# HeyWeCome/WhisprRec

Measured on AMD Instinct MI355X. Metric: BPR training triplets/sec, higher is better.
Workload: dtype f32; 1 GPU; BPRMF emb_size=64, synthetic 1000000 users x 1000000 items (uniform ids), batch 65536, SGD l2=0, plan build in timed region; batch=65536, emb_size=64, optimizer=SGD, plan_chunk_batches=64, tables=single GPU, step_stream=whisprrec_amd.hip_ops.PipelinedSgd, plan=group plan (no per-batch sort: flags + lists of the shared rows, wr_group.hip), chained_step_launch=True, plan_build=on a side stream, beside the steps of the chunk before

## Files before the change

whisprrec_amd/csrc/wr_group.hip:

```cpp
#include "wr_common.h"
#include <hip/hip_ext.h>

#include <algorithm>

namespace wr {

constexpr int kGpThreads = 1024;
constexpr unsigned kGpRangeBits = 18;
constexpr int kGpWords = 1 << (kGpRangeBits - 5);
constexpr int kGpCap = 8192;
constexpr int kGpBins = 4096;
constexpr int kGpMaxBin = 256;
constexpr int kGpMaxRanges = 8;
constexpr int64_t kGpMaxBatch = 1 << 17;
constexpr int kGpLongRun = 64;
constexpr int kGpMetaWords = 16;
#ifndef WR_GP_DBG
#define WR_GP_DBG 0
#endif

struct GroupLayout {
    int64_t nb, B, fw;
    int R_u, R_i, cap_u, cap_i;
    unsigned mask_u, mask_i, hbits_u, hbits_i;
    int64_t flags, ucnt, icnt, ul_row, ul_src, il_row, il_src, total;
    int64_t zero_words;
};

static inline int ranges_for(int64_t n_rows, unsigned *mask, unsigned *hbits, int *cap) {
    unsigned bits = kGpRangeBits;
    while (bits < kGpRangeBits + 3 && (int64_t(1) << bits) < n_rows) ++bits;
    *mask = (1u << bits) - 1u;
    *hbits = bits;
    const int R = 1 << (bits - kGpRangeBits);
    *cap = kGpCap;
    return R;
}

static bool group_layout(int64_t n, int64_t B, int64_t n_users, int64_t n_items, GroupLayout &L) {
    if (n <= 0 || n >= (int64_t(1) << 31) || B <= 0 || B > kGpMaxBatch) return false;
    if (n_users <= 0 || n_users >= (int64_t(1) << 31) || n_items <= 0 || n_items >= (int64_t(1) << 31)) return false;
    L.nb = (n + B - 1) / B;
    L.B = B;
    L.fw = (B + 31) / 32;
    L.R_u = ranges_for(n_users, &L.mask_u, &L.hbits_u, &L.cap_u);
    L.R_i = ranges_for(n_items, &L.mask_i, &L.hbits_i, &L.cap_i);
    L.flags = kGpMetaWords;
    L.ucnt = L.flags + L.nb * L.fw * 4;
    L.icnt = L.ucnt + align_up(L.nb * L.R_u, 4);
    L.zero_words = L.icnt + align_up(L.nb * L.R_i, 4);
    L.ul_row = L.zero_words;
    L.ul_src = L.ul_row + L.nb * L.R_u * (int64_t)L.cap_u;
    L.il_row = L.ul_src + L.nb * L.R_u * (int64_t)L.cap_u;
    L.il_src = L.il_row + L.nb * L.R_i * (int64_t)L.cap_i;
    L.total = L.il_src + L.nb * L.R_i * (int64_t)L.cap_i;
    return true;
}

struct GpDev {
    int *meta;
    unsigned *flags;
    int *ucnt, *icnt;
    int *ul_row, *ul_src, *il_row, *il_src;
    int R_u, R_i, cap_u, cap_i;
    unsigned mask_u, mask_i, hbits_u, hbits_i;
    int fw;
};

static inline GpDev group_dev(int32_t *plan, const GroupLayout &L) {
    return GpDev{plan, reinterpret_cast<unsigned *>(plan + L.flags), plan + L.ucnt, plan + L.icnt, plan + L.ul_row,
                 plan + L.ul_src, plan + L.il_row, plan + L.il_src, L.R_u, L.R_i, L.cap_u, L.cap_i, L.mask_u, L.mask_i,
                 L.hbits_u, L.hbits_i, (int)L.fw};
}

template <typename F>
__device__ __forceinline__ void gp_scan(const int *__restrict__ a, int cnt, F f) {
    if ((reinterpret_cast<uintptr_t>(a) & 15u) == 0) {
        const int n4 = cnt >> 2;
        const int4 *a4 = reinterpret_cast<const int4 *>(a);
        int i = threadIdx.x;
        for (; i + 3 * kGpThreads < n4; i += 4 * kGpThreads) {
            int4 v[4];
#pragma unroll
            for (int q = 0; q < 4; ++q) v[q] = a4[i + q * kGpThreads];
#pragma unroll
            for (int q = 0; q < 4; ++q) {
                const int at = 4 * (i + q * kGpThreads);
                f(v[q].x, at);
                f(v[q].y, at + 1);
                f(v[q].z, at + 2);
                f(v[q].w, at + 3);
            }
        }
        for (; i < n4; i += kGpThreads) {
            const int4 v = a4[i];
            f(v.x, 4 * i);
            f(v.y, 4 * i + 1);
            f(v.z, 4 * i + 2);
            f(v.w, 4 * i + 3);
        }
        for (int j = (n4 << 2) + threadIdx.x; j < cnt; j += kGpThreads) f(a[j], j);
    } else {
        for (int j = threadIdx.x; j < cnt; j += kGpThreads) f(a[j], j);
    }
}

__global__ __launch_bounds__(kGpThreads) void group_plan_kernel(const int *__restrict__ u, const int *__restrict__ p,
                                                                 const int *__restrict__ n, int64_t n_total, int B, int nb,
                                                                 int n_users, int n_items, GpDev L) {
    extern __shared__ __attribute__((aligned(16))) unsigned gp_lds[];
    unsigned *seen = gp_lds;
    unsigned long long *keys = reinterpret_cast<unsigned long long *>(gp_lds);
    unsigned *multi = gp_lds + 2 * kGpCap;
    unsigned *f0 = multi + kGpWords, *f1 = f0 + L.fw, *f2 = f1 + L.fw;
    int &n_list = *reinterpret_cast<int *>(f2 + L.fw);
    const int per = L.R_u + L.R_i;
    const unsigned lb = xcd_contiguous_id(blockIdx.x, gridDim.x);
    const int b = (int)(lb / (unsigned)per), rr = (int)(lb % (unsigned)per);
    const bool item = rr >= L.R_u;
    const unsigned r = (unsigned)(item ? rr - L.R_u : rr);
    const int64_t base = (int64_t)b * B;
    const int Bb = (int)((base + B <= n_total) ? B : (n_total - base));
    const unsigned n_rows = (unsigned)(item ? n_items : n_users);
    const unsigned mask = item ? L.mask_i : L.mask_u;
    const unsigned rb = (item ? L.hbits_i : L.hbits_u) - kGpRangeBits, rsel = (1u << rb) - 1u;
    for (int i = threadIdx.x; i < kGpWords; i += kGpThreads) {
        seen[i] = 0u;
        multi[i] = 0u;
    }
    for (int i = threadIdx.x; i < 3 * L.fw; i += kGpThreads) f0[i] = 0u;
    if (threadIdx.x == 0) n_list = 0;
    __syncthreads();
    auto mark = [&](int row, int) {
        if ((unsigned)row >= n_rows) {
            L.meta[0] = 1;
            return;
        }
        const unsigned h = (unsigned)row & mask;
        if ((h & rsel) != r) return;
        const unsigned bit = h >> rb, m = 1u << (bit & 31u);
        const unsigned old = atomicOr(&seen[bit >> 5], m);
        if (old & m) atomicOr(&multi[bit >> 5], m);
    };
    if (!(WR_GP_DBG & 8)) {
        if (item) {
            gp_scan(p + base, Bb, mark);
            gp_scan(n + base, Bb, mark);
        } else {
            gp_scan(u + base, Bb, mark);
        }
    }
    __syncthreads();
    auto several = [&](int row) -> bool {
        const unsigned h = (unsigned)row & mask;
        if ((h & rsel) != r) return false;
        const unsigned bit = h >> rb;
        return (multi[bit >> 5] >> (bit & 31u)) & 1u;
    };
    auto append = [&](int row, unsigned src) {
        const int pos = atomicAdd(&n_list, 1);
        if (pos < kGpCap) keys[pos] = ((unsigned long long)(unsigned)row << 32) | src;
    };
    if (!(WR_GP_DBG & 2)) {
        const bool next = b + 1 < nb && !(WR_GP_DBG & 16);
        const int64_t nbase = base + B;
        const int Bn = next ? (int)((nbase + B <= n_total) ? B : (n_total - nbase)) : 0;
        auto defer = [&](int row, int t) {
            if (several(row)) atomicOr(&f2[t >> 5], 1u << (t & 31));
        };
        if (item) {
            gp_scan(p + base, Bb, [&](int row, int t) {
                if (several(row)) {
                    atomicOr(&f0[t >> 5], 1u << (t & 31));
                    append(row, (unsigned)t << 1);
                }
            });
            gp_scan(n + base, Bb, [&](int row, int t) {
                if (several(row)) {
                    atomicOr(&f1[t >> 5], 1u << (t & 31));
                    append(row, ((unsigned)t << 1) | 1u);
                }
            });
            gp_scan(p + nbase, Bn, defer);
            gp_scan(n + nbase, Bn, defer);
        } else {
            gp_scan(u + base, Bb, [&](int row, int t) {
                if (several(row)) {
                    atomicOr(&f0[t >> 5], 1u << (t & 31));
                    append(row, (unsigned)t << 1);
                }
            });
            gp_scan(u + nbase, Bn, defer);
        }
    }
    __syncthreads();
    if (!(WR_GP_DBG & 4)) {
        unsigned *fb = L.flags + (int64_t)b * L.fw * 4;
        for (int w = threadIdx.x; w < L.fw; w += kGpThreads) {
            if (f0[w]) __hip_atomic_fetch_or(fb + 4 * w + (item ? 1 : 0), f0[w], __ATOMIC_RELAXED, __HIP_MEMORY_SCOPE_AGENT);
            if (item && f1[w]) __hip_atomic_fetch_or(fb + 4 * w + 2, f1[w], __ATOMIC_RELAXED, __HIP_MEMORY_SCOPE_AGENT);
            if (f2[w])
                __hip_atomic_fetch_or(fb + 4 * (L.fw + w) + 3, f2[w], __ATOMIC_RELAXED, __HIP_MEMORY_SCOPE_AGENT);
        }
    }
    const int cap = item ? L.cap_i : L.cap_u, R = item ? L.R_i : L.R_u;
    int m = n_list;
    if (m > cap) {
        if (threadIdx.x == 0) L.meta[1] = 1;
        m = cap;
    }
    int *cnt = reinterpret_cast<int *>(multi);
    unsigned short *out16 = reinterpret_cast<unsigned short *>(multi + kGpBins);
    int *wave_tot = reinterpret_cast<int *>(f0);
    auto bin_of = [&](unsigned long long k) -> int { return (int)(((((unsigned)(k >> 32)) & mask) >> rb) & (kGpBins - 1)); };
    int *lrow = (item ? L.il_row : L.ul_row) + ((int64_t)b * R + r) * cap, *lsrc = (item ? L.il_src : L.ul_src) + ((int64_t)b * R + r) * cap;
    __syncthreads();
    for (int i = threadIdx.x; i < kGpBins; i += kGpThreads) cnt[i] = 0;
    __syncthreads();
    if (!(WR_GP_DBG & 1)) {
        for (int j = threadIdx.x; j < m; j += kGpThreads) atomicAdd(&cnt[bin_of(keys[j])], 1);
        __syncthreads();
        constexpr int kOwn = kGpBins / kGpThreads;
        const int c0 = (int)threadIdx.x * kOwn;
        int local = 0;
#pragma unroll
        for (int j = 0; j < kOwn; ++j) local += cnt[c0 + j];
        int incl = local;
#pragma unroll
        for (int d = 1; d < 64; d <<= 1) {
            const int v = __shfl_up(incl, d, 64);
            if ((int)(threadIdx.x & 63) >= d) incl += v;
        }
        if ((threadIdx.x & 63) == 63) wave_tot[threadIdx.x >> 6] = incl;
        __syncthreads();
        int run = incl - local;
        for (int w = 0; w < (int)(threadIdx.x >> 6); ++w) run += wave_tot[w];
#pragma unroll
        for (int j = 0; j < kOwn; ++j) {
            const int c = cnt[c0 + j];
            cnt[c0 + j] = run;
            run += c;
        }
        __syncthreads();
        for (int j = threadIdx.x; j < m; j += kGpThreads) out16[atomicAdd(&cnt[bin_of(keys[j])], 1)] = (unsigned short)j;
        __syncthreads();
        for (int j = threadIdx.x; j < m; j += kGpThreads) {
            const unsigned long long k = keys[j];
            const int bin = bin_of(k);
            const int lo = bin ? cnt[bin - 1] : 0, hi = cnt[bin];
            if (hi - lo > kGpMaxBin) {
                L.meta[1] = 1;
                continue;
            }
            int pos = lo, same = 0;
            for (int jj = lo; jj < hi; ++jj) {
                const unsigned long long o = keys[out16[jj]];
                pos += o < k ? 1 : 0;
                same += (unsigned)(o >> 32) == (unsigned)(k >> 32) ? 1 : 0;
            }
            if (same > kGpLongRun) L.meta[2] = 1;
            lrow[pos] = (int)(k >> 32);
            lsrc[pos] = (int)(unsigned)k;
        }
    } else {
        for (int j = threadIdx.x; j < m; j += kGpThreads) {
            lrow[j] = (int)(keys[j] >> 32);
            lsrc[j] = (int)(unsigned)keys[j];
        }
    }
    if (threadIdx.x == 0) (item ? L.icnt : L.ucnt)[(int64_t)b * R + r] = m;
}

__global__ __launch_bounds__(kBlock) void narrow_ids_kernel(const int64_t *__restrict__ u, const int64_t *__restrict__ p,
                                                             const int64_t *__restrict__ n, int *__restrict__ u32,
                                                             int *__restrict__ p32, int *__restrict__ n32, int64_t cnt) {
    const int64_t i = (int64_t)blockIdx.x * kBlock + threadIdx.x;
    if (i >= cnt) return;
    const int64_t a = u[i], b = p[i], c = n[i];
    u32[i] = (a >= 0 && a < (int64_t(1) << 31)) ? (int)a : -1;
    p32[i] = (b >= 0 && b < (int64_t(1) << 31)) ? (int)b : -1;
    n32[i] = (c >= 0 && c < (int64_t(1) << 31)) ? (int)c : -1;
}

constexpr int kGsTile = 32;
constexpr int kGsAhead = 8;
constexpr int kGsShards = 64;
constexpr int kGsShardStride = 16;
constexpr int kGsStepWords = kGsShards * kGsShardStride;
constexpr int kGsDefChunk = 32;
constexpr int kGsLdsInts = 1024 + 8;
constexpr unsigned kGsSpinLimit = 1u << 22;

struct GsBatch {
    const int *u, *p, *n;
    const uint4 *flags;
    const int *ul_row, *ul_src, *ul_cnt, *il_row, *il_src, *il_cnt;
    int B, R_u, R_i, cap_u, cap_i;
};

struct GsArgs {
    float *U, *I;
    int D;
    float lr;
    GsBatch cur;
    float *Z, *ZU, *partials;
    float denom;
    GsBatch prev;
    const float *Zp, *ZUp, *partials_prev;
    int n_partials_prev;
    float denom_prev;
    float *loss_prev;
    int nA, nIT, nUT, nDS, tiles_at, side_at;
    int chained;
    unsigned *done, *timeout;
    float *Gs;
    int nL;
};

template <int NV>
__device__ __forceinline__ Row<NV> row_zero() {
    Row<NV> r;
#pragma unroll
    for (int k = 0; k < NV; ++k) r.v[k] = make_float4(0.f, 0.f, 0.f, 0.f);
    return r;
}

template <int T, int NV, bool FULL>
__device__ __forceinline__ void gs_single(const GsArgs &a, int t, int u, int p, int n, bool us, bool ps, bool ns, int lane,
                                          float &terms) {
    const Row<NV> ur = load_row<T, NV, FULL>(a.U, u, a.D, lane);
    const Row<NV> pr = load_row<T, NV, FULL>(a.I, p, a.D, lane);
    const Row<NV> nr = load_row<T, NV, FULL>(a.I, n, a.D, lane);
    const float sp = team_sum<T>(dot_partial<NV>(ur, pr));
    const float sn = team_sum<T>(dot_partial<NV>(ur, nr));
    float term, c;
    bpr_terms(sp, sn, a.denom, term, c);
    terms += term;
    Row<NV> g, z;
#pragma unroll
    for (int k = 0; k < NV; ++k) {
        g.v[k] = make_float4(c * (pr.v[k].x - nr.v[k].x), c * (pr.v[k].y - nr.v[k].y), c * (pr.v[k].z - nr.v[k].z),
                             c * (pr.v[k].w - nr.v[k].w));
        z.v[k] = make_float4(c * ur.v[k].x, c * ur.v[k].y, c * ur.v[k].z, c * ur.v[k].w);
    }
    const float lr = a.lr;
    if (!us) {
        Row<NV> w;
#pragma unroll
        for (int k = 0; k < NV; ++k)
            w.v[k] = make_float4(ur.v[k].x - lr * g.v[k].x, ur.v[k].y - lr * g.v[k].y, ur.v[k].z - lr * g.v[k].z,
                                 ur.v[k].w - lr * g.v[k].w);
        store_row<T, NV, FULL>(a.U, u, a.D, lane, w);
    } else {
        store_row<T, NV, FULL>(a.ZU, t, a.D, lane, g);
    }
    if (!ps) {
        if (a.Gs != nullptr && p >= a.nL) {
            store_row<T, NV, FULL>(a.Gs, p - a.nL, a.D, lane, z);
        } else {
            Row<NV> w;
#pragma unroll
            for (int k = 0; k < NV; ++k)
                w.v[k] = make_float4(pr.v[k].x - lr * z.v[k].x, pr.v[k].y - lr * z.v[k].y, pr.v[k].z - lr * z.v[k].z,
                                     pr.v[k].w - lr * z.v[k].w);
            store_row<T, NV, FULL>(a.I, p, a.D, lane, w);
        }
    }
    if (!ns) {
        if (a.Gs != nullptr && n >= a.nL) {
            Row<NV> zn;
#pragma unroll
            for (int k = 0; k < NV; ++k) zn.v[k] = make_float4(-z.v[k].x, -z.v[k].y, -z.v[k].z, -z.v[k].w);
            store_row<T, NV, FULL>(a.Gs, n - a.nL, a.D, lane, zn);
        } else {
            Row<NV> w;
#pragma unroll
            for (int k = 0; k < NV; ++k)
                w.v[k] = make_float4(nr.v[k].x - lr * (-z.v[k].x), nr.v[k].y - lr * (-z.v[k].y), nr.v[k].z - lr * (-z.v[k].z),
                                     nr.v[k].w - lr * (-z.v[k].w));
            store_row<T, NV, FULL>(a.I, n, a.D, lane, w);
        }
    }
    if (ps || ns) store_row<T, NV, FULL>(a.Z, t, a.D, lane, z);
}

__device__ __forceinline__ void gs_wait_tiles(const GsArgs &a) {
    if (threadIdx.x < 64) {
        const int j = (int)threadIdx.x;
        const int n_sig = a.nIT + a.nUT;
        const unsigned want = j < kGsShards ? (unsigned)((n_sig - j + kGsShards - 1) / kGsShards) : 0u;
        const unsigned *shard = a.done + (j < kGsShards ? j : 0) * kGsShardStride;
        unsigned spins = 0;
        for (;;) {
            const bool ok = __hip_atomic_load(shard, __ATOMIC_RELAXED, __HIP_MEMORY_SCOPE_AGENT) >= want;
            if (__all(ok)) break;
            __builtin_amdgcn_s_sleep(8);
            if (++spins > kGsSpinLimit) {
                if (j == 0) __hip_atomic_store(a.timeout, 1u, __ATOMIC_RELAXED, __HIP_MEMORY_SCOPE_AGENT);
                break;
            }
        }
        __builtin_amdgcn_fence(__ATOMIC_ACQUIRE, "agent");
        asm volatile("s_waitcnt vmcnt(0)" ::: "memory");
    }
    __syncthreads();
}

__device__ __forceinline__ bool gs_tile_of(const int *__restrict__ cnt, int R, int cap, int q, int &seg, int &e0, int &len) {
    int c[kGpMaxRanges];
#pragma unroll
    for (int s = 0; s < kGpMaxRanges; ++s) c[s] = cnt[s < R ? s : 0];
    asm volatile("" : "+v"(c[0]), "+v"(c[1]), "+v"(c[2]), "+v"(c[3]), "+v"(c[4]), "+v"(c[5]), "+v"(c[6]), "+v"(c[7]));
#pragma unroll
    for (int s = 0; s < kGpMaxRanges; ++s)
        if (s >= R) c[s] = 0;
    bool found = false;
#pragma unroll
    for (int s = 0; s < kGpMaxRanges; ++s) {
        const int cs = min(c[s], cap);
        const int nt = (cs + kGsTile - 1) / kGsTile;
        if (!found && q < nt) {
            seg = s;
            e0 = q * kGsTile;
            len = cs;
            found = true;
        }
        if (!found) q -= nt;
    }
    return found;
}

struct GsTile {
    const int *lrow, *lsrc;
    int e0, len;
    int er, es, before;
};

__device__ __forceinline__ void gs_tile_fetch(GsTile &tl, const int *__restrict__ l_row, const int *__restrict__ l_src, int seg,
                                              int cap, int e0, int len, int B) {
    tl.lrow = l_row + (int64_t)seg * cap;
    tl.lsrc = l_src + (int64_t)seg * cap;
    tl.e0 = e0;
    tl.len = len;
    tl.er = -1;
    tl.es = 0;
    tl.before = -1;
    const int e = e0 + (int)threadIdx.x;
    if (threadIdx.x < kGsTile + kGsAhead && e < len) {
        tl.er = tl.lrow[e];
        tl.es = tl.lsrc[e];
    }
    if (threadIdx.x == 0 && e0 > 0) tl.before = tl.lrow[e0 - 1];
}

template <int T, int NV, bool FULL, bool WT>
__device__ __forceinline__ void gs_tile_finish(float *__restrict__ W, int D, float lr, int B, const float *__restrict__ Z,
                                               const GsTile &tl, int *__restrict__ lds, float *__restrict__ Gs = nullptr,
                                               int nL = 0) {
    int *rows_t = lds, *src_t = rows_t + (kGsTile + kGsAhead), *heads = src_t + (kGsTile + kGsAhead);
    int &n_heads = heads[kGsTile];
    constexpr int TEAMS = kBlock / T;
    const int lane = threadIdx.x % T;
    __syncthreads();
    if (threadIdx.x == 0) n_heads = 0;
    if (threadIdx.x < kGsTile + kGsAhead) {
        rows_t[threadIdx.x] = tl.er;
        src_t[threadIdx.x] = min(max(tl.es, 0), 2 * B - 1);
    }
    __syncthreads();
    if (threadIdx.x < kGsTile) {
        const int r = rows_t[threadIdx.x];
        const int bf = threadIdx.x == 0 ? tl.before : rows_t[threadIdx.x - 1];
        if (r >= 0 && bf != r) heads[atomicAdd(&n_heads, 1)] = threadIdx.x;
    }
    __syncthreads();
    const int nh = n_heads;
    for (int h = threadIdx.x / T; h < nh; h += TEAMS) {
        const int j0 = heads[h];
        const int r = rows_t[j0];
        const bool slot = Gs != nullptr && r >= nL;
        Row<NV> ir = row_zero<NV>();
        if (!slot) ir = load_row<T, NV, FULL>(W, r, D, lane);
        const int s0 = src_t[j0];
        const bool two = rows_t[j0 + 1] == r;
        const int s1 = src_t[j0 + 1];
        const Row<NV> z0 = load_row<T, NV, FULL>(Z, s0 >> 1, D, lane);
        Row<NV> z1 = row_zero<NV>();
        if (two) z1 = load_row<T, NV, FULL>(Z, s1 >> 1, D, lane);
        Row<NV> g;
        const float g0 = (s0 & 1) ? -1.0f : 1.0f, g1 = (s1 & 1) ? -1.0f : 1.0f;
#pragma unroll
        for (int k = 0; k < NV; ++k) {
            g.v[k].x = fmaf(g0, z0.v[k].x, 0.f);
            g.v[k].y = fmaf(g0, z0.v[k].y, 0.f);
            g.v[k].z = fmaf(g0, z0.v[k].z, 0.f);
            g.v[k].w = fmaf(g0, z0.v[k].w, 0.f);
        }
        if (two) {
#pragma unroll
            for (int k = 0; k < NV; ++k) {
                g.v[k].x = fmaf(g1, z1.v[k].x, g.v[k].x);
                g.v[k].y = fmaf(g1, z1.v[k].y, g.v[k].y);
                g.v[k].z = fmaf(g1, z1.v[k].z, g.v[k].z);
                g.v[k].w = fmaf(g1, z1.v[k].w, g.v[k].w);
            }
            auto add_z = [&](int src) {
                const Row<NV> z = load_row<T, NV, FULL>(Z, src >> 1, D, lane);
                const float sgn = (src & 1) ? -1.0f : 1.0f;
#pragma unroll
                for (int k = 0; k < NV; ++k) {
                    g.v[k].x = fmaf(sgn, z.v[k].x, g.v[k].x);
                    g.v[k].y = fmaf(sgn, z.v[k].y, g.v[k].y);
                    g.v[k].z = fmaf(sgn, z.v[k].z, g.v[k].z);
                    g.v[k].w = fmaf(sgn, z.v[k].w, g.v[k].w);
                }
            };
            int j = j0 + 2;
            for (; j < kGsTile + kGsAhead && rows_t[j] == r; ++j) add_z(src_t[j]);
            if (j == kGsTile + kGsAhead)
                for (int e = tl.e0 + j; e < tl.len && tl.lrow[e] == r; ++e) add_z(min(max(tl.lsrc[e], 0), 2 * B - 1));
        }
        if (slot) {
            store_row<T, NV, FULL>(Gs, r - nL, D, lane, g);
            continue;
        }
        Row<NV> wv;
#pragma unroll
        for (int k = 0; k < NV; ++k)
            wv.v[k] = make_float4(ir.v[k].x - lr * g.v[k].x, ir.v[k].y - lr * g.v[k].y, ir.v[k].z - lr * g.v[k].z,
                                  ir.v[k].w - lr * g.v[k].w);
        if constexpr (WT) store_row_wt<T, NV, FULL>(W, r, D, lane, wv);
        else store_row<T, NV, FULL>(W, r, D, lane, wv);
    }
}

#ifndef WR_GS_WAVES
#define WR_GS_WAVES 8
#endif
#ifndef WR_GS_DBG
#define WR_GS_DBG 0
#endif

template <int T, int NV, bool FULL, bool WT>
__device__ __forceinline__ void gs_list_tiles(float *__restrict__ W, int D, float lr, const int *__restrict__ l_row,
                                              const int *__restrict__ l_src, const int *__restrict__ l_cnt, int R, int cap,
                                              int B, const float *__restrict__ Z, int w, int nw, int *__restrict__ lds,
                                              float *__restrict__ Gs = nullptr, int nL = 0) {
    for (int q = w;; q += nw) {
        int seg, e0, len;
        if (!gs_tile_of(l_cnt, R, cap, q, seg, e0, len)) break;
        GsTile tl;
        gs_tile_fetch(tl, l_row, l_src, seg, cap, e0, len, B);
        gs_tile_finish<T, NV, FULL, WT>(W, D, lr, B, Z, tl, lds, Gs, nL);
    }
}

template <int T, int NV, bool FULL>
__global__ __launch_bounds__(kBlock, NV == 1 ? WR_GS_WAVES : 1) void bprmf_group_step(GsArgs a) {
    __shared__ float scratch[kBlock / 64];
    __shared__ __attribute__((aligned(16))) int lds[kGsLdsInts];
    constexpr int TEAMS = kBlock / T;
    const int lane = threadIdx.x % T;
    int b = (int)blockIdx.x;
    if (b >= a.tiles_at && b < a.tiles_at + a.nIT + a.nUT) {
        const int w = b - a.tiles_at;
        const bool wt = a.nA > 0;
        if (!(WR_GS_DBG & 1)) {
            if (w < a.nIT) {
                if (wt) gs_list_tiles<T, NV, FULL, true>(a.I, a.D, a.lr, a.prev.il_row, a.prev.il_src, a.prev.il_cnt, a.prev.R_i, a.prev.cap_i,
                                                         a.prev.B, a.Zp, w, a.nIT, lds, a.Gs, a.nL);
                else gs_list_tiles<T, NV, FULL, false>(a.I, a.D, a.lr, a.prev.il_row, a.prev.il_src, a.prev.il_cnt, a.prev.R_i, a.prev.cap_i,
                                                       a.prev.B, a.Zp, w, a.nIT, lds, a.Gs, a.nL);
            } else {
                if (wt) gs_list_tiles<T, NV, FULL, true>(a.U, a.D, a.lr, a.prev.ul_row, a.prev.ul_src, a.prev.ul_cnt, a.prev.R_u, a.prev.cap_u,
                                                         a.prev.B, a.ZUp, w - a.nIT, a.nUT, lds);
                else gs_list_tiles<T, NV, FULL, false>(a.U, a.D, a.lr, a.prev.ul_row, a.prev.ul_src, a.prev.ul_cnt, a.prev.R_u, a.prev.cap_u,
                                                       a.prev.B, a.ZUp, w - a.nIT, a.nUT, lds);
            }
        }
        if (wt) {
            asm volatile("s_waitcnt vmcnt(0)" ::: "memory");
            __syncthreads();
            if (threadIdx.x == 0)
                __hip_atomic_fetch_add(a.done + (w % kGsShards) * kGsShardStride, 1u, __ATOMIC_RELAXED, __HIP_MEMORY_SCOPE_AGENT);
        }
        if (w == 0 && a.loss_prev != nullptr) {
            const float s0 = strided_partial_sum(a.partials_prev, a.n_partials_prev);
            const float s = block_sum(s0, scratch);
            if (threadIdx.x == 0) a.loss_prev[0] = s / a.denom_prev;
        }
        return;
    }
    if (b >= a.tiles_at) b -= a.nIT + a.nUT;
    float terms = 0.f;
    int slot;
    if (b >= a.side_at && b < a.side_at + a.nDS) {
        const int w = b - a.side_at;
        int *dl = lds, &total_s = lds[kGsDefChunk * 32];
        const int fw = (a.cur.B + 31) / 32;
        const int per = (fw + a.nDS - 1) / a.nDS;
        const int w_end = min(fw, (w + 1) * per);
        bool waited = false;
        for (int c0 = w * per; c0 < w_end; c0 += kGsDefChunk) {
            const int wi = c0 + (int)threadIdx.x;
            unsigned m = 0u, us = 0u, ps = 0u, ns = 0u;
            if (threadIdx.x < kGsDefChunk && wi < w_end) {
                const uint4 f = a.cur.flags[wi];
                m = f.w;
                us = f.x;
                ps = f.y;
                ns = f.z;
            }
            int cnt = __popc(m), incl = cnt;
#pragma unroll
            for (int d = 1; d < 64; d <<= 1) {
                const int v = __shfl_up(incl, d, 64);
                if ((int)(threadIdx.x & 63) >= d) incl += v;
            }
            if (threadIdx.x == 63) total_s = incl;
            int at = incl - cnt;
            while (m) {
                const int bit = __ffs(m) - 1;
                m &= m - 1;
                dl[at++] = ((wi * 32 + bit) << 3) | (((us >> bit) & 1u) ? 4 : 0) | (((ps >> bit) & 1u) ? 1 : 0) |
                           (((ns >> bit) & 1u) ? 2 : 0);
            }
            __syncthreads();
            const int total = (WR_GS_DBG & 2) ? 0 : total_s;
            const int e0 = (int)threadIdx.x / T, e1 = e0 + TEAMS;
            int t0 = 0, u0 = 0, p0 = 0, n0 = 0, t1 = 0, u1 = 0, p1 = 0, n1 = 0;
            if (e0 < total) {
                t0 = min(dl[e0] >> 3, a.cur.B - 1);
                u0 = a.cur.u[t0];
                p0 = a.cur.p[t0];
                n0 = a.cur.n[t0];
            }
            if (e1 < total) {
                t1 = min(dl[e1] >> 3, a.cur.B - 1);
                u1 = a.cur.u[t1];
                p1 = a.cur.p[t1];
                n1 = a.cur.n[t1];
            }
            if (!waited) {
                if (!(WR_GS_DBG & 4)) gs_wait_tiles(a);
                waited = true;
            }
            if (e0 < total) gs_single<T, NV, FULL>(a, t0, u0, p0, n0, dl[e0] & 4, dl[e0] & 1, dl[e0] & 2, lane, terms);
            if (e1 < total) gs_single<T, NV, FULL>(a, t1, u1, p1, n1, dl[e1] & 4, dl[e1] & 1, dl[e1] & 2, lane, terms);
            for (int e = e1 + TEAMS; e < total; e += TEAMS) {
                const int t = min(dl[e] >> 3, a.cur.B - 1);
                gs_single<T, NV, FULL>(a, t, a.cur.u[t], a.cur.p[t], a.cur.n[t], dl[e] & 4, dl[e] & 1, dl[e] & 2, lane, terms);
            }
            __syncthreads();
        }
        slot = a.nA + w;
    } else {
        if (b >= a.side_at) b -= a.nDS;
        const int t = b * TEAMS + (int)threadIdx.x / T;
        const int tc = min(t, a.cur.B - 1);
        uint4 f = a.cur.flags[tc >> 5];
        int u = a.cur.u[tc], p = a.cur.p[tc], n = a.cur.n[tc];
#if WR_GS_DBG & 8
        f = make_uint4(0u, 0u, 0u, 0u);
#endif
        asm volatile("" : "+v"(u), "+v"(p), "+v"(n), "+v"(f.x), "+v"(f.y), "+v"(f.z), "+v"(f.w));
        const unsigned bit = 1u << (t & 31);
        if (t < a.cur.B && !(a.chained && (f.w & bit)))
            gs_single<T, NV, FULL>(a, t, u, p, n, f.x & bit, f.y & bit, f.z & bit, lane, terms);
        slot = b;
    }
    if (lane != 0) terms = 0.f;
    const float sum = block_sum(terms, scratch);
    if (threadIdx.x == 0) a.partials[slot] = sum;
}

static inline int64_t gs_ws_one(int64_t B, int32_t D) {
    const int64_t nA = (B + teams_per_block(D) - 1) / teams_per_block(D);
    return 2 * align_up(B * (int64_t)D * 4, 256) + align_up((nA + 512) * 4, 256);
}

#ifndef WR_GS_TILES_AT
#define WR_GS_TILES_AT 0
#endif
#ifndef WR_GS_SIDE_AT
#define WR_GS_SIDE_AT 12
#endif
#ifndef WR_GS_NUT
#define WR_GS_NUT 256
#endif
#ifndef WR_GS_NDS
#define WR_GS_NDS 64
#endif
#ifndef WR_GS_NIT
#define WR_GS_NIT 1024
#endif

struct GroupRun {
    TablePair tabs;
    const int32_t *u, *p, *n, *plan;
    int64_t n_triplets, batch_size, plan_words, workspace_bytes, sync_words;
    BatchRange range;
    float lr, *loss_out;
    void *const *events;
    void *workspace;
    uint32_t *sync;
    int n_cu;
    float *grad_slots;
    int64_t n_local_items, global_batch;
    hipStream_t stream;
};

template <int T, int NV, bool FULL>
static int32_t launch_group_steps(const GroupRun &g, const GroupLayout &L, const GpDev &G) {
    const int32_t D = g.tabs.D;
    const int64_t n_batches = g.range.n_batches, global_batch = g.global_batch;
    uint32_t *const sync = g.sync;
    const int64_t B = L.B;
    const int64_t ws_one = gs_ws_one(B, D), zb = align_up(B * (int64_t)D * 4, 256);
    char *ws = reinterpret_cast<char *>(g.workspace);
    float *Zs[2] = {reinterpret_cast<float *>(ws), reinterpret_cast<float *>(ws + ws_one)};
    float *ZUs[2] = {reinterpret_cast<float *>(ws + zb), reinterpret_cast<float *>(ws + ws_one + zb)};
    float *Ps[2] = {reinterpret_cast<float *>(ws + 2 * zb), reinterpret_cast<float *>(ws + ws_one + 2 * zb)};
    constexpr int TEAMS = kBlock / T;
    WR_HIP(hipMemsetAsync(sync, 0, (size_t)(n_batches * kGsStepWords) * 4, g.stream));
    uint32_t *timeout = sync + (g.sync_words - 4);
    int nDS = WR_GS_NDS;
    while (nDS > g.n_cu / 4 && nDS > 1) nDS >>= 1;
    auto batch_of = [&](int64_t b) {
        const int64_t off = b * B;
        const int Bk = (int)batch_len(g.n_triplets, B, b);
        return GsBatch{g.u + off, g.p + off, g.n + off, reinterpret_cast<const uint4 *>(G.flags + b * L.fw * 4),
                       G.ul_row + b * L.R_u * (int64_t)L.cap_u, G.ul_src + b * L.R_u * (int64_t)L.cap_u, G.ucnt + b * L.R_u,
                       G.il_row + b * L.R_i * (int64_t)L.cap_i, G.il_src + b * L.R_i * (int64_t)L.cap_i, G.icnt + b * L.R_i,
                       Bk, L.R_u, L.R_i, L.cap_u, L.cap_i};
    };
    auto ev = [&](int64_t k, int j) { return g.events ? reinterpret_cast<hipEvent_t>(g.events[2 * k + j]) : (hipEvent_t) nullptr; };
    int n_partials_prev = 0;
    for (int64_t k = 0; k <= n_batches; ++k) {
        GsArgs a{};
        a.U = g.tabs.U;
        a.I = g.tabs.I;
        a.D = D;
        a.lr = g.lr;
        a.done = sync + (k < n_batches ? k : 0) * kGsStepWords;
        a.timeout = timeout;
        a.Gs = g.grad_slots;
        a.nL = (int)g.n_local_items;
        const bool have_cur = k < n_batches, have_prev = k > 0;
        if (have_cur) {
            a.cur = batch_of(g.range.first_batch + k);
            a.Z = Zs[k & 1];
            a.ZU = ZUs[k & 1];
            a.partials = Ps[k & 1];
            a.denom = global_batch > 0 ? (float)global_batch : (float)a.cur.B;
            a.nA = (int)((a.cur.B + TEAMS - 1) / TEAMS);
            a.nDS = have_prev ? nDS : 0;
            a.chained = have_prev ? 1 : 0;
        }
        if (have_prev) {
            a.prev = batch_of(g.range.first_batch + k - 1);
            a.Zp = Zs[(k - 1) & 1];
            a.ZUp = ZUs[(k - 1) & 1];
            a.partials_prev = Ps[(k - 1) & 1];
            a.n_partials_prev = n_partials_prev;
            a.denom_prev = global_batch > 0 ? (float)global_batch : (float)a.prev.B;
            a.loss_prev = at_or_null(g.loss_out, k - 1);
            a.nIT = (int)std::min<int64_t>(WR_GS_NIT, (2 * B + kGsTile - 1) / kGsTile + L.R_i);
            a.nUT = (int)std::min<int64_t>(WR_GS_NUT, (B + kGsTile - 1) / kGsTile + L.R_u);
        }
        a.tiles_at = (int)((int64_t)a.nA * WR_GS_TILES_AT / 16);
        a.side_at = std::max(a.tiles_at, (int)((int64_t)a.nA * WR_GS_SIDE_AT / 16));
        const dim3 grid((unsigned)(a.nA + a.nIT + a.nUT + a.nDS));
        hipEvent_t e0 = have_cur ? ev(k, 0) : nullptr, e1 = have_cur ? ev(k, 1) : nullptr;
        if (e0 != nullptr || e1 != nullptr)
            hipExtLaunchKernelGGL((bprmf_group_step<T, NV, FULL>), grid, dim3(kBlock), 0, g.stream, e0, e1, 0, a);
        else
            hipLaunchKernelGGL((bprmf_group_step<T, NV, FULL>), grid, dim3(kBlock), 0, g.stream, a);
        WR_LAUNCH_CHECK("bprmf_group_step");
        n_partials_prev = a.nA + a.nDS;
    }
    return WR_OK;
}

static int32_t check_group_plan(const char *entry, const GroupRun &g, GroupLayout &L) {
    int32_t rc;
    if ((rc = check_whole_lines(entry, whole_lines(g.tabs.U, g.tabs.I, g.tabs.D), g.tabs.D)) != WR_OK) return rc;
    WR_REQUIRE(group_layout(g.n_triplets, g.batch_size, g.tabs.n_users, g.tabs.n_items, L), WR_E_RANGE,
               "group plan not applicable to n=%lld, batch=%lld", (long long)g.n_triplets, (long long)g.batch_size);
    WR_REQUIRE(g.plan_words >= L.total, WR_E_WORKSPACE, "group plan: %lld words < %lld", (long long)g.plan_words, (long long)L.total);
    return WR_OK;
}

static int32_t run_group(const char *entry, GroupRun &g, const GroupLayout &L, int64_t sync_batches) {
    int32_t rc;
    if ((rc = check_workspace(entry, g.workspace, g.workspace_bytes, 2 * gs_ws_one(g.batch_size, g.tabs.D))) != WR_OK) return rc;
    if ((rc = check_sync_words(entry, g.sync, g.sync_words, sync_batches * kGsStepWords + 4)) != WR_OK) return rc;
    if (g.range.n_batches == 0) return WR_OK;
    if (g.n_cu == 0 && (rc = device_cu_count(&g.n_cu)) != WR_OK) return rc;
    const GpDev G = group_dev(const_cast<int32_t *>(g.plan), L);
#define WR_CALL_GS(T_, NV_, FULL_) return launch_group_steps<T_, NV_, FULL_>(g, L, G)
    WR_DISPATCH_D(g.tabs.D, WR_CALL_GS);
#undef WR_CALL_GS
    return WR_OK;
}

}

using namespace wr;

extern "C" {

int64_t wr_group_plan_words(int64_t n_triplets, int64_t batch_size, int64_t n_users, int64_t n_items) {
    GroupLayout L;
    if (!group_layout(n_triplets, batch_size, n_users, n_items, L)) return 0;
    return L.total;
}

int32_t wr_group_plan_layout(int64_t n_triplets, int64_t batch_size, int64_t n_users, int64_t n_items, int64_t *out) {
    WR_REQUIRE(out != nullptr, WR_E_NULL, "out is NULL");
    GroupLayout L;
    WR_REQUIRE(group_layout(n_triplets, batch_size, n_users, n_items, L), WR_E_RANGE,
               "group plan not applicable to n=%lld, batch=%lld", (long long)n_triplets, (long long)batch_size);
    const int64_t v[16] = {L.nb, L.fw, L.R_u, L.R_i, (int64_t)L.mask_u, (int64_t)L.mask_i, L.flags, L.ucnt, L.icnt, L.ul_row,
                           L.ul_src, L.il_row, L.il_src, L.total, L.cap_u, L.cap_i};
    for (int i = 0; i < 16; ++i) out[i] = v[i];
    return WR_OK;
}

int32_t wr_narrow_ids_i64(const int64_t *u, const int64_t *p, const int64_t *n, int32_t *u32, int32_t *p32, int32_t *n32,
                          int64_t count, void *stream_) {
    WR_REQUIRE(u && p && n && u32 && p32 && n32, WR_E_NULL, "index arrays must not be NULL");
    WR_REQUIRE(count >= 0 && count < (int64_t(1) << 40), WR_E_SHAPE, "count out of range");
    if (count == 0) return WR_OK;
    hipLaunchKernelGGL(narrow_ids_kernel, dim3((unsigned)((count + kBlock - 1) / kBlock)), dim3(kBlock), 0,
                       reinterpret_cast<hipStream_t>(stream_), u, p, n, u32, p32, n32, count);
    WR_LAUNCH_CHECK("narrow_ids_kernel");
    return WR_OK;
}

int32_t wr_group_plan_build(const int32_t *u, const int32_t *p, const int32_t *n, int64_t n_triplets, int64_t batch_size,
                            int64_t n_users, int64_t n_items, int32_t *plan, int64_t plan_words, void *stream_) {
    WR_REQUIRE(u && p && n && plan, WR_E_NULL, "index arrays / plan must not be NULL");
    GroupLayout L;
    WR_REQUIRE(group_layout(n_triplets, batch_size, n_users, n_items, L), WR_E_RANGE,
               "group plan not applicable to n=%lld, batch=%lld", (long long)n_triplets, (long long)batch_size);
    WR_REQUIRE(aligned16(plan) && plan_words >= L.total, WR_E_WORKSPACE, "group plan: %lld words < %lld", (long long)plan_words,
               (long long)L.total);
    WR_REQUIRE(L.nb * (L.R_u + L.R_i) < (int64_t(1) << 31), WR_E_SHAPE, "group plan: too many batches in one plan");
    hipStream_t stream = reinterpret_cast<hipStream_t>(stream_);
    WR_HIP(hipMemsetAsync(plan, 0, (size_t)L.zero_words * 4, stream));
    const size_t lds = (size_t)(2 * kGpCap + kGpWords + 3 * L.fw + 4) * 4;
    static bool attr_set = false;
    if (!attr_set) {
        WR_HIP(hipFuncSetAttribute(reinterpret_cast<const void *>(group_plan_kernel), hipFuncAttributeMaxDynamicSharedMemorySize,
                                   (int)((2 * kGpCap + kGpWords + 3 * ((kGpMaxBatch + 31) / 32) + 4) * 4)));
        attr_set = true;
    }
    const GpDev G = group_dev(plan, L);
    hipLaunchKernelGGL(group_plan_kernel, dim3((unsigned)(L.nb * (L.R_u + L.R_i))), dim3(kGpThreads), lds, stream, u, p, n,
                       n_triplets, (int)batch_size, (int)L.nb, (int)n_users, (int)n_items, G);
    WR_LAUNCH_CHECK("group_plan_kernel");
    return WR_OK;
}

int64_t wr_bprmf_group_workspace_bytes(int64_t batch_size, int32_t D) { return 2 * gs_ws_one(batch_size, D); }

int64_t wr_bprmf_group_sync_words(int64_t n_batches) { return n_batches < 0 ? WR_E_SHAPE : (n_batches + 1) * kGsStepWords + 4; }

int32_t wr_bprmf_group_supported(const float *user_tab, const float *item_tab, int32_t D) {
    return (user_tab && item_tab && D >= 4 && D <= 1024 && D % 4 == 0 && whole_lines(user_tab, item_tab, D)) ? 1 : 0;
}

int32_t wr_bprmf_run_sgd_group(float *user_tab, int64_t n_users, float *item_tab, int64_t n_items, int32_t D,
                               const int32_t *u, const int32_t *p, const int32_t *n, int64_t n_triplets, int64_t batch_size,
                               const int32_t *plan, int64_t plan_words, int64_t first_batch, int64_t n_batches, float lr,
                               float *loss_out, void *const *events, void *workspace, int64_t workspace_bytes, int32_t *sync,
                               int64_t sync_words, void *stream) {
    GroupRun g{};
    g.tabs = TablePair{user_tab, item_tab, n_users, n_items, D};
    g.u = u; g.p = p; g.n = n; g.n_triplets = n_triplets; g.batch_size = batch_size;
    g.plan = plan; g.plan_words = plan_words;
    g.range = BatchRange{first_batch, n_batches};
    g.lr = lr; g.loss_out = loss_out; g.events = events;
    g.workspace = workspace; g.workspace_bytes = workspace_bytes;
    g.sync = reinterpret_cast<uint32_t *>(sync); g.sync_words = sync_words;
    g.stream = reinterpret_cast<hipStream_t>(stream);
    int32_t rc;
    GroupLayout L;
    if ((rc = check_tables(g.tabs)) != WR_OK) return rc;
    WR_REQUIRE(u && p && n && plan && sync, WR_E_NULL, "index arrays / plan / sync words must not be NULL");
    if ((rc = check_group_plan("wr_bprmf_run_sgd_group", g, L)) != WR_OK) return rc;
    WR_REQUIRE(first_batch >= 0 && n_batches >= 0 && first_batch + n_batches <= L.nb, WR_E_SHAPE,
               "batches [%lld,%lld) exceed the plan's %lld", (long long)first_batch, (long long)(first_batch + n_batches),
               (long long)L.nb);
    return run_group("wr_bprmf_run_sgd_group", g, L, n_batches + 1);
}

int32_t wr_bprmf_shard_step_group(float *user_shard, int64_t n_user_rows, float *item_ext, int64_t n_ext_rows,
                                  int64_t n_local_items, int32_t D, const int32_t *vu, const int32_t *vp, const int32_t *vn,
                                  int64_t n_triplets, int64_t batch_size, const int32_t *plan, int64_t plan_words, int64_t batch,
                                  int64_t global_batch, float lr, float *grad_slots, float *loss_partial, void *workspace,
                                  int64_t workspace_bytes, int32_t *sync, int64_t sync_words, void *stream) {
    GroupRun g{};
    g.tabs = TablePair{user_shard, item_ext, n_user_rows, n_ext_rows, D};
    g.u = vu; g.p = vp; g.n = vn; g.n_triplets = n_triplets; g.batch_size = batch_size;
    g.plan = plan; g.plan_words = plan_words;
    g.range = BatchRange{batch, 1};
    g.lr = lr; g.loss_out = loss_partial;
    g.workspace = workspace; g.workspace_bytes = workspace_bytes;
    g.sync = reinterpret_cast<uint32_t *>(sync); g.sync_words = sync_words;
    g.n_cu = 256;
    g.grad_slots = grad_slots; g.n_local_items = n_local_items; g.global_batch = global_batch;
    g.stream = reinterpret_cast<hipStream_t>(stream);
    int32_t rc;
    GroupLayout L;
    if ((rc = check_tables(g.tabs, "user_shard", "item_ext")) != WR_OK) return rc;
    WR_REQUIRE(vu && vp && vn && plan && sync && grad_slots, WR_E_NULL, "index arrays / plan / sync words / grad_slots must not be NULL");
    WR_REQUIRE(aligned16(grad_slots), WR_E_ALIGN, "grad_slots is not 16-byte aligned");
    WR_REQUIRE(n_local_items >= 0 && n_local_items <= n_ext_rows, WR_E_SHAPE, "n_local_items %lld outside [0, %lld]",
               (long long)n_local_items, (long long)n_ext_rows);
    if ((rc = check_group_plan("wr_bprmf_shard_step_group", g, L)) != WR_OK) return rc;
    WR_REQUIRE(batch >= 0 && batch < L.nb, WR_E_SHAPE, "batch %lld outside the plan's %lld", (long long)batch, (long long)L.nb);
    WR_REQUIRE(global_batch >= batch_size, WR_E_SHAPE, "global_batch %lld < local batch %lld", (long long)global_batch,
               (long long)batch_size);
    return run_group("wr_bprmf_shard_step_group", g, L, 2);
}

}
```

Baseline: 2.589 billion triplets/s.

## Split long row runs across all teams of the workgroup with LDS staging

Rows in a tile whose run of contributions reaches at least kGsCoopMin entries are pulled out of the per-team serial loop. They go to a cooperative path where every team loads a slice of the Z rows into an LDS staging buffer, and the owner team reduces from it. The aim is to stop a single team from serially walking long runs of duplicate rows while the other teams sit idle, which mainly matters for hot rows. In exchange it adds block-wide barriers per chunk and a larger LDS footprint, which may lower occupancy. Under uniform ids long runs are rare, so the new path may seldom fire.

```diff
diff --git a/whisprrec_amd/csrc/wr_group.hip b/whisprrec_amd/csrc/wr_group.hip
--- a/whisprrec_amd/csrc/wr_group.hip
+++ b/whisprrec_amd/csrc/wr_group.hip
@@ -288,7 +288,25 @@
 constexpr int kGsShardStride = 16;
 constexpr int kGsStepWords = kGsShards * kGsShardStride;
 constexpr int kGsDefChunk = 32;
+#ifndef WR_GS_COOP
+#define WR_GS_COOP 1
+#endif
+#ifndef WR_GS_COOP_MIN
+#define WR_GS_COOP_MIN 8
+#endif
+constexpr int kGsCoopMin = WR_GS_COOP_MIN;
+constexpr int kGsLongAt = 120;
+constexpr int kGsSignAt = 160;
+constexpr int kGsStageAt = 256;
+constexpr int kGsStageBytes = 8192;
+constexpr int kGsStageMax = 64;
+#if WR_GS_COOP
+constexpr int kGsLdsInts = kGsStageAt + kGsStageBytes / 4;
+#else
 constexpr int kGsLdsInts = 1024 + 8;
+#endif
+static_assert(kGsLdsInts >= 1024 + 8 && 2 * (kGsTile + kGsAhead) + kGsTile + 1 <= kGsLongAt && kGsLongAt + kGsTile + 1 <= kGsSignAt &&
+              kGsSignAt + kGsStageMax <= kGsStageAt, "LDS layout of the tile workgroups");
 constexpr unsigned kGsSpinLimit = 1u << 22;
 
 struct GsBatch {
@@ -453,16 +471,141 @@
     if (threadIdx.x == 0 && e0 > 0) tl.before = tl.lrow[e0 - 1];
 }
 
+template <class P>
+__device__ __forceinline__ P *gs_uniform(P *p) {
+    const unsigned long long v = reinterpret_cast<unsigned long long>(p);
+    const unsigned lo = __builtin_amdgcn_readfirstlane((unsigned)v), hi = __builtin_amdgcn_readfirstlane((unsigned)(v >> 32));
+    return reinterpret_cast<P *>(((unsigned long long)hi << 32) | lo);
+}
+
+template <int T, int NV>
+constexpr int gs_stage_rows() {
+    constexpr int fit = kGsStageBytes / (T * NV * 16), two = 2 * (kBlock / T);
+    return fit < two ? (fit < kGsStageMax ? fit : kGsStageMax) : (two < kGsStageMax ? two : kGsStageMax);
+}
+
+template <int T, int NV, bool FULL, bool WT>
+__device__ __forceinline__ void gs_tile_long_runs(float *__restrict__ W, int D, float lr, int B, const float *__restrict__ Z,
+                                                  const GsTile &tl, int *__restrict__ lds, int nl, float *__restrict__ Gs, int nL) {
+    constexpr int TEAMS = kBlock / T, S = gs_stage_rows<T, NV>(), WIN = kGsTile + kGsAhead;
+    constexpr bool TWO = S > TEAMS;
+    static_assert(S >= 1 && S <= kGsStageMax && S <= 2 * TEAMS && S * T * NV * 16 <= kGsStageBytes, "staging buffer");
+    const int *rows_t = lds, *src_t = rows_t + WIN, *longs = lds + kGsLongAt;
+    float *sgn_s = reinterpret_cast<float *>(lds + kGsSignAt);
+    float4 *stage = reinterpret_cast<float4 *>(lds + kGsStageAt);
+    const int lane = threadIdx.x % T, tm = threadIdx.x / T;
+    const int e0 = __builtin_amdgcn_readfirstlane(tl.e0), len = __builtin_amdgcn_readfirstlane(tl.len);
+    const int *lrow = gs_uniform(tl.lrow), *lsrc = gs_uniform(tl.lsrc);
+    nl = __builtin_amdgcn_readfirstlane(nl);
+    for (int h = 0; h < nl; ++h) {
+        const int j0 = __builtin_amdgcn_readfirstlane(longs[h]);
+        const int r = __builtin_amdgcn_readfirstlane(rows_t[j0]);
+        const bool owner = tm == h % TEAMS;
+        const bool slot = Gs != nullptr && r >= nL;
+        Row<NV> ir = row_zero<NV>();
+        if (owner && !slot) ir = load_row<T, NV, FULL>(W, r, D, lane);
+        Row<NV> g = row_zero<NV>();
+        Row<NV> za = row_zero<NV>(), zb = row_zero<NV>();
+        float sa = 0.f, sb = 0.f;
+        auto request = [&](int i0) {
+            const int ja = j0 + i0 + tm, jb = ja + TEAMS;
+            int ra = -1, ca = 0, rb = -1, cb = 0;
+            if (tm < S) {
+                if (ja < WIN) {
+                    ra = rows_t[ja];
+                    ca = src_t[ja];
+                } else if (e0 + ja < len) {
+                    ra = lrow[e0 + ja];
+                    ca = lsrc[e0 + ja];
+                }
+            }
+            if (TWO && tm + TEAMS < S) {
+                if (jb < WIN) {
+                    rb = rows_t[jb];
+                    cb = src_t[jb];
+                } else if (e0 + jb < len) {
+                    rb = lrow[e0 + jb];
+                    cb = lsrc[e0 + jb];
+                }
+            }
+            ca = min(max(ca, 0), 2 * B - 1);
+            cb = min(max(cb, 0), 2 * B - 1);
+            sa = ra != r ? 0.f : (ca & 1) ? -1.0f : 1.0f;
+            sb = rb != r ? 0.f : (cb & 1) ? -1.0f : 1.0f;
+            if (sa != 0.f) za = load_row<T, NV, FULL>(Z, ca >> 1, D, lane);
+            if (TWO && sb != 0.f) zb = load_row<T, NV, FULL>(Z, cb >> 1, D, lane);
+        };
+        request(0);
+        for (int i0 = 0;; i0 += S) {
+            if (tm < S) {
+                if (sa != 0.f) {
+#pragma unroll
+                    for (int k = 0; k < NV; ++k) stage[(tm * NV + k) * T + lane] = za.v[k];
+                }
+                if (lane == 0) sgn_s[tm] = sa;
+            }
+            if (TWO && tm + TEAMS < S) {
+                if (sb != 0.f) {
+#pragma unroll
+                    for (int k = 0; k < NV; ++k) stage[((tm + TEAMS) * NV + k) * T + lane] = zb.v[k];
+                }
+                if (lane == 0) sgn_s[tm + TEAMS] = sb;
+            }
+            __syncthreads();
+            const int wl = (int)(threadIdx.x & 63);
+            const unsigned long long in_run = __ballot(wl < S && sgn_s[wl < S ? wl : 0] != 0.f);
+            const int nv = ~in_run == 0ull ? 64 : __ffsll((long long)~in_run) - 1;
+            const bool more = nv == S;
+            if (more) request(i0 + S);
+            if (owner) {
+#pragma unroll 2
+                for (int s = 0; s < nv; ++s) {
+                    const float sgn = sgn_s[s];
+#pragma unroll
+                    for (int k = 0; k < NV; ++k) {
+                        const float4 z = stage[(s * NV + k) * T + lane];
+                        g.v[k].x = fmaf(sgn, z.x, g.v[k].x);
+                        g.v[k].y = fmaf(sgn, z.y, g.v[k].y);
+                        g.v[k].z = fmaf(sgn, z.z, g.v[k].z);
+                        g.v[k].w = fmaf(sgn, z.w, g.v[k].w);
+                    }
+                }
+            }
+            __syncthreads();
+            if (!more) break;
+        }
+        if (!owner) continue;
+        if (slot) {
+            store_row<T, NV, FULL>(Gs, r - nL, D, lane, g);
+            continue;
+        }
+        Row<NV> wv;
+#pragma unroll
+        for (int k = 0; k < NV; ++k)
+            wv.v[k] = make_float4(ir.v[k].x - lr * g.v[k].x, ir.v[k].y - lr * g.v[k].y, ir.v[k].z - lr * g.v[k].z,
+                                  ir.v[k].w - lr * g.v[k].w);
+        if constexpr (WT) store_row_wt<T, NV, FULL>(W, r, D, lane, wv);
+        else store_row<T, NV, FULL>(W, r, D, lane, wv);
+    }
+}
+
 template <int T, int NV, bool FULL, bool WT>
 __device__ __forceinline__ void gs_tile_finish(float *__restrict__ W, int D, float lr, int B, const float *__restrict__ Z,
                                                const GsTile &tl, int *__restrict__ lds, float *__restrict__ Gs = nullptr,
                                                int nL = 0) {
     int *rows_t = lds, *src_t = rows_t + (kGsTile + kGsAhead), *heads = src_t + (kGsTile + kGsAhead);
     int &n_heads = heads[kGsTile];
+#if WR_GS_COOP
+    int *longs = lds + kGsLongAt;
+    int &n_long = longs[kGsTile];
+#endif
     constexpr int TEAMS = kBlock / T;
     const int lane = threadIdx.x % T;
     __syncthreads();
     if (threadIdx.x == 0) n_heads = 0;
+#if WR_GS_COOP
+    if (threadIdx.x == 0) n_long = 0;
+#endif
     if (threadIdx.x < kGsTile + kGsAhead) {
         rows_t[threadIdx.x] = tl.er;
         src_t[threadIdx.x] = min(max(tl.es, 0), 2 * B - 1);
@@ -471,7 +614,15 @@
     if (threadIdx.x < kGsTile) {
         const int r = rows_t[threadIdx.x];
         const int bf = threadIdx.x == 0 ? tl.before : rows_t[threadIdx.x - 1];
+#if WR_GS_COOP
+        static_assert(kGsCoopMin >= 2 && kGsCoopMin <= kGsAhead, "the test of a long run stays inside the staged window");
+        if (r >= 0 && bf != r) {
+            if (rows_t[threadIdx.x + kGsCoopMin] == r) longs[atomicAdd(&n_long, 1)] = threadIdx.x;
+            else heads[atomicAdd(&n_heads, 1)] = threadIdx.x;
+        }
+#else
         if (r >= 0 && bf != r) heads[atomicAdd(&n_heads, 1)] = threadIdx.x;
+#endif
     }
     __syncthreads();
     const int nh = n_heads;
@@ -517,8 +668,10 @@
             };
             int j = j0 + 2;
             for (; j < kGsTile + kGsAhead && rows_t[j] == r; ++j) add_z(src_t[j]);
+#if !WR_GS_COOP
             if (j == kGsTile + kGsAhead)
                 for (int e = tl.e0 + j; e < tl.len && tl.lrow[e] == r; ++e) add_z(min(max(tl.lsrc[e], 0), 2 * B - 1));
+#endif
         }
         if (slot) {
             store_row<T, NV, FULL>(Gs, r - nL, D, lane, g);
@@ -532,6 +685,10 @@
         if constexpr (WT) store_row_wt<T, NV, FULL>(W, r, D, lane, wv);
         else store_row<T, NV, FULL>(W, r, D, lane, wv);
     }
+#if WR_GS_COOP
+    const int nl = n_long;
+    if (nl > 0) gs_tile_long_runs<T, NV, FULL, WT>(W, D, lr, B, Z, tl, lds, nl, Gs, nL);
+#endif
 }
 
 #ifndef WR_GS_WAVES
```

New measurement: 2.582 billion triplets/s. No clear change (-0.3%).
